# arihantb2/direct_lidar_odometry

Measured on AMD Instinct MI355X. Metric: gicp_iterations_per_sec, higher is better.
Workload: dtype f64

## Files before the change

### direct_lidar_odometry_amd/csrc/ngicp_align.h

```cpp
#pragma once

namespace {

std::mutex& persist_mutex(int device) {
  static std::mutex m[64];
  return m[(unsigned)device % 64u];
}

int pass_impl() {
  static const int impl = std::getenv("NGICP_PASS_IMPL") ? std::atoi(std::getenv("NGICP_PASS_IMPL")) : 0;
  return impl;
}

const char* robust_unsupported_switch(const ngicp* h) {
  if (pass_impl() == 1) return "NGICP_PASS_IMPL=1";
  if (const char* s = std::getenv("NGICP_FUSED")) if (std::atoi(s) != 0) return "NGICP_FUSED";
  if (const char* s = std::getenv("NGICP_QUEUE")) if (std::atoi(s) != 0) return "NGICP_QUEUE";
  if (h->persist) return "NGICP_PERSIST";
  if (h->head) return "NGICP_HEAD";
  return nullptr;
}
void refuse_if_robust(const ngicp* h, const char* entry) {
  if (h->robust_kind != NGICP_ROBUST_NONE)
    throw ArgError{NGICP_ERR_ARG, std::string(entry) + ": not available with a robust kernel set (ngicp_set_robust_kernel(h, NGICP_ROBUST_NONE, 0) turns it off)"};
}
void refuse_robust_under_switch(const ngicp* h, const char* entry) {
  if (h->robust_kind == NGICP_ROBUST_NONE) return;
  if (const char* sw = robust_unsupported_switch(h))
    throw ArgError{NGICP_ERR_ARG, std::string(entry) + ": the robust kernel has no instantiation of the pass variant " + sw + " selects (unset it, or ngicp_set_robust_kernel(h, NGICP_ROBUST_NONE, 0))"};
}
void fill_robust(const ngicp* h, int& kind, double& c, double& c2) {
  kind = h->robust_kind;
  c = h->robust_width;
  c2 = h->robust_width * h->robust_width;
}

void launch_pass(ngicp* h, const PassArgs& a, int nblocks, hipStream_t s, hipEvent_t start = nullptr, hipEvent_t stop = nullptr) {
  static const int force = std::getenv("NGICP_PASS_WPS") ? std::atoi(std::getenv("NGICP_PASS_WPS")) : 0;
  const int impl = pass_impl();
  const bool four = force ? force == 4 : nblocks > 2 * h->pass_slots;
  if (impl == 1) {
    PassArgs b = a;
    b.fused = 0;
    int need = kStGrowMax;
    if (h->p.max_corr_dist < 1e30) need = (int)std::ceil(h->p.max_corr_dist / (double)a.grid.h);
    b.stage_grow = std::max(1, std::min(kStGrowMax, need));
    if (force ? force == 4 : true)
      hipExtLaunchKernelGGL((k_gicp_pass_st<4>), dim3(nblocks), dim3(256), 0, s, start, stop, 0, b);
    else
      hipExtLaunchKernelGGL((k_gicp_pass_st<3>), dim3(nblocks), dim3(256), 0, s, start, stop, 0, b);
    return;
  }
  static const int queue_env = std::getenv("NGICP_QUEUE") ? std::atoi(std::getenv("NGICP_QUEUE")) : 0;
  if (queue_env && !a.fused && !(a.mode & 4) && !a.dbg_stamps && !a.dbg_span && !a.dbg_qstats) {
    if (four)
      hipExtLaunchKernelGGL((k_gicp_queue<2, 4>), dim3((unsigned)std::min(nblocks, h->queue_slots[1])), dim3(256), 0, s, start, stop, 0, a);
    else
      hipExtLaunchKernelGGL((k_gicp_queue<2, 3>), dim3((unsigned)std::min(nblocks, h->queue_slots[0])), dim3(256), 0, s, start, stop, 0, a);
    return;
  }
  if (a.fused) {
    if (four)
      hipExtLaunchKernelGGL((k_gicp_pass<2, 4, true>), dim3(nblocks), dim3(256), 0, s, start, stop, 0, a);
    else
      hipExtLaunchKernelGGL((k_gicp_pass<2, 3, true>), dim3(nblocks), dim3(256), 0, s, start, stop, 0, a);
    return;
  }
  if (a.robust_kind != NGICP_ROBUST_NONE) {
    if (four)
// ... 114 lines not shown
  s.cfg.lm_init_lambda_factor = h->p.lm_init_lambda_factor;
  s.partials = a.partials;
  s.nblocks = nblocks;
  s.grp_order = order_buf[h->order_sel];
  s.grp_cost = a.grp_cost;
  s.trace = own_buffers ? h->trace.as<double>() : nullptr;
  s.max_trace_rows = max_rows;
  s.mode = 0;
  s.sums_out = nullptr;
  s.dbg_stamps = nullptr;
  s.progress_host = nullptr;
  s.final_host = nullptr;
  s.order_valid = order_flag[h->order_sel];
  s.t_first = nullptr;
  s.persist = 0;
  s.pass_ticks = nullptr;
  s.st_out = nullptr;
  s.nrows = 0;
  a.crow_in = nullptr;
  a.crow_out = nullptr;
  a.cluster_ticket = nullptr;
  a.done_flag = nullptr;
  c.nblocks = nblocks;
  if (!own_buffers) return;
  h->stats.lanes_per_query = 2;
  h->stats.voxel_size = a.grid.h;
  h->stats.grid_dims[0] = a.grid.nx;
  h->stats.grid_dims[1] = a.grid.ny;
  h->stats.grid_dims[2] = a.grid.nz;
}
// ... 47 lines not shown
      for (int cc = 0; cc < 6; ++cc) hessian[cc * 6 + rr] = r.final_H[rr * 6 + cc];
  if (r.lm_failed) std::fprintf(stderr, "lm not converged!!\n");
}

void publish_alignment(ngicp* h, const LmState& st, float loop_ms, float* aligned, size_t out_stride) {
  store_result(st.hot, h->final_T, &h->converged, &h->nr_iterations, h->final_hessian);
  h->trace_host.clear();
  h->trace_rows_dev = (size_t)st.hot.n_trace;
  if (aligned) download_transformed(h, *h->src.dev, h->final_T, aligned, out_stride);
  if (st.hot.have_lin) h->hook_valid = 2;
  ngicp_stats& s = h->stats;
  s.loop_ms = loop_ms;
  s.passes = st.hot.passes;
  s.outer_iterations = st.hot.nr_iterations + 1;
  s.lm_trials = st.hot.n_trace;
  s.mean_candidates = st.hot.passes > 0 ? st.hot.cand_total / ((double)st.hot.passes * (double)h->src.dev->n) : 0.0;
  s.valid_fraction = st.hot.passes > 0 ? st.hot.valid_total / ((double)st.hot.passes * (double)h->src.dev->n) : 0.0;
  s.pass_ms_total = 0.0;
  s.passes_timed = 0;
}

void sum_event_pass_times(ngicp* h, long passes) {
  if (!h->profiling) return;
  ngicp_stats& s = h->stats;
  const long timed = std::min<long>(passes, (long)h->prof_events.size() / 2);
  int counted = 0;
  for (long i = h->prof_stride / 2; i < timed; i += h->prof_stride) {
    float ms = 0.f;
    if (hipEventElapsedTime(&ms, h->prof_events[2 * i], h->prof_events[2 * i + 1]) == hipSuccess) {
      s.pass_ms_total += ms;
      ++counted;
    }
// ... 63 lines not shown
}

void end_alignment(ngicp* h, Alignment& al, float* aligned, size_t out_stride, bool event_times = true) {
  publish_alignment(h, al.st, al.loop_ms, aligned, out_stride);
  if (event_times) sum_event_pass_times(h, al.st.hot.passes);
  ngicp_stats& s = h->stats;
  s.n_src = (long long)h->src.dev->n;
  s.n_tgt = rolling_active(h) ? (long long)h->roll.n_vox : (long long)h->tgt.dev->n;
  s.host_wait_spins = (long long)al.spins;
  s.align_ms = now_ms() - al.t_begin;
}

void set_pass_mode(const ngicp* h, PassArgs& a) {
  a.mode = (h->p.optimizer == NGICP_OPT_GAUSS_NEWTON) ? 2 : 3;
  if (h->prev_staged_fraction < 0.0 || h->prev_staged_fraction >= 0.12) a.mode |= 32;
}

bool install_xcd_order(ngicp* h, LoopCtx& c) {
  static const bool xcd_order = std::getenv("NGICP_ORDER") && std::string(std::getenv("NGICP_ORDER")) == "xcd";
  if (!xcd_order) return false;
  const int nb = c.nblocks, per = (nb + 7) / 8;
  std::vector<int> ord((size_t)nb);
  std::vector<int> lists[8];
  for (int g = 0; g < nb; ++g) lists[std::min(7, g / per)].push_back(g);
  size_t taken[8] = {0, 0, 0, 0, 0, 0, 0, 0};
  int b = 0;
  for (int placed = 0; placed < nb; ++b) {
    int x = b % 8;
    if (taken[x] >= lists[x].size()) {
      x = 0;
// ... 184 lines not shown
  pa.sa.persist = 1;
  HIP_TRY(hipMemsetAsync(pa.ticket, 0, sizeof(int), h->stream));
  HIP_TRY(hipMemsetAsync(h->gen_lines.p, 0, (size_t)kGenLines * kGenStride * sizeof(int), h->stream));
  hipExtLaunchKernelGGL((k_gicp_persist<2, 3>), dim3((unsigned)std::min(c.nblocks, h->persist_slots)), dim3(256), 0, h->stream, start, stop, 0, pa);
}

void do_align(ngicp* h, const float guess[16], float* aligned, size_t out_stride) {
  refuse_robust_under_switch(h, "ngicp_align");
  Alignment al;
  reset_results(h);
  LoopCtx c;
  prepare_loop(h, c);
  if (!(h->order_src == h->src.dev.get() && h->order_groups == c.sa.nblocks)) HIP_TRY(hipMemsetAsync(h->order_flag.p, 0, 4 * sizeof(int), h->stream));
  const bool xcd_order = install_xcd_order(h, c);
  set_pass_mode(h, c.pa);
  if (const char* dbg = std::getenv("NGICP_DEBUG_MODE")) c.pa.mode |= (std::atoi(dbg) & (8 | 16));
  begin_alignment(h, al, guess, c.sa, c.pa.t_first);
  const DebugDumps dbg = debug_begin(h, c);
  static const bool fused_env = std::getenv("NGICP_FUSED") && std::atoi(std::getenv("NGICP_FUSED")) != 0;
  if (fused_env && pass_impl() == 0) {
    c.pa.fused = 1;
    c.pa.sa = c.sa;
    HIP_TRY(hipMemsetAsync(c.pa.ticket, 0, sizeof(int), h->stream));
  }
  const long max_p = max_passes(h->p);
  const bool plain = h->p.max_iter > 0 && pass_impl() == 0 && !c.pa.fused && !xcd_order && !dbg.span_path && !dbg.qstat_path && !c.sa.dbg_stamps;
  const bool want_persist = h->persist && plain && h->persist_slots > 0 && !dbg.stamp_path && max_p + 1 <= kMaxPersistPasses;
  const bool persist_done = want_persist && align_persistent(h, c, al, max_p);
  const bool head_mode = h->head && plain && !persist_done && c.nblocks <= 2 * h->pass_slots;
  static const bool persist_one = std::getenv("NGICP_PERSIST_ONE") != nullptr;
  if (persist_done) {
  } else if (head_mode) {
    head_begin(h);
    feed_alignment(h, al, max_p + 1, [&](long i, hipEvent_t start, hipEvent_t stop) { launch_head(h, c, i, start, stop); });
    if ((al.st.hot.passes + 1) & 1) HIP_TRY(hipMemcpyAsync(h->state.p, h->state_alt.p, sizeof(LmState), hipMemcpyDeviceToDevice, h->stream));
  } else if (persist_one && h->persist_slots > 0 && max_p + 1 <= kMaxPersistPasses) {
    feed_alignment(h, al, max_p, [&](long i, hipEvent_t start, hipEvent_t stop) { launch_persist_one(h, c, i, start, stop); });
  } else {
    feed_alignment(h, al, max_p, [&](long, hipEvent_t start, hipEvent_t stop) {
      launch_pass(h, c.pa, c.nblocks, h->stream, start, stop);
      if (!c.pa.fused) hipLaunchKernelGGL(k_lm_solve, dim3(1), dim3(kSolveThreads), 0, h->stream, c.sa);
    });
  }
  HIP_TRY(hipGetLastError());
  debug_end(h, c, dbg);
  end_alignment(h, al, aligned, out_stride, !persist_done);
  ngicp_stats& s = h->stats;
  h->order_src = h->src.dev.get();
  h->order_groups = c.sa.nblocks;
  s.staged_fraction = al.st.hot.passes > 0 ? al.st.hot.staged_total / ((double)al.st.hot.passes * (double)h->src.dev->n) : 0.0;
  if (al.st.hot.passes > 1) h->prev_staged_fraction = s.staged_fraction;
  if (persist_done && h->profiling) sum_tick_pass_times(h, al.st.hot);
}

struct VoxelCtx {
  VoxelPassArgs pa;
  SolveArgs sa;
  int nblocks;
};

void launch_voxel_pass(ngicp* h, const VoxelCtx& c, hipEvent_t start = nullptr, hipEvent_t stop = nullptr) {
  const dim3 grid((unsigned)c.nblocks), block(kVoxBlock);
  if (c.pa.robust_kind != NGICP_ROBUST_NONE) {
    switch (c.pa.nbr) {
      case NGICP_VOX_DIRECT1: hipExtLaunchKernelGGL(k_vgicp_pass<true>, grid, block, 0, h->stream, start, stop, 0, c.pa); break;
      case NGICP_VOX_DIRECT7: hipExtLaunchKernelGGL((k_vgicp_pass_n<7, true>), grid, block, 0, h->stream, start, stop, 0, c.pa); break;
// ... 344 lines not shown
```

### direct_lidar_odometry_amd/csrc/ngicp_api.hip

```cpp
#include "../../include/ngicp.h"

#include <hip/hip_runtime.h>
#include <hip/hip_ext.h>

#include <algorithm>
#include <atomic>
#include <chrono>
#include <cmath>
#include <cstdio>
#include <cstdlib>
#include <cstring>
#include <limits>
#include <memory>
#include <mutex>
#include <sched.h>
#include <string>
#include <vector>

#include "ngicp_pass.h"
#include "ngicp_cloudops.h"
#include "ngicp_filters.h"
#include "ngicp_query.h"
#include "ngicp_range.h"
#include "ngicp_batch.h"
// ... 543 lines not shown
      int cus = 0, per_cu = 0;
      HIP_TRY(hipDeviceGetAttribute(&cus, hipDeviceAttributeMultiprocessorCount, device));
      HIP_TRY(hipOccupancyMaxActiveBlocksPerMultiprocessor(&per_cu, k_gicp_pass<2, 3>, 256, 0));
      h->pass_slots = std::max(1, cus) * std::max(1, per_cu);
      int per_cu_p = 0;
      if (hipOccupancyMaxActiveBlocksPerMultiprocessor(&per_cu_p, k_gicp_persist<2, 3>, 256, 0) == hipSuccess) h->persist_slots = std::max(0, cus) * std::max(0, per_cu_p);
      int q3 = 0, q4 = 0;
      if (hipOccupancyMaxActiveBlocksPerMultiprocessor(&q3, k_gicp_queue<2, 3>, 256, 0) == hipSuccess && q3 > 0) h->queue_slots[0] = cus * q3;
      if (hipOccupancyMaxActiveBlocksPerMultiprocessor(&q4, k_gicp_queue<2, 4>, 256, 0) == hipSuccess && q4 > 0) h->queue_slots[1] = cus * q4;
      int coop = 0;
      if (hipDeviceGetAttribute(&coop, hipDeviceAttributeCooperativeLaunch, device) != hipSuccess || !coop) h->persist_slots = 0;
    }
    HIP_TRY(hipHostMalloc(reinterpret_cast<void**>(&h->pin_ticks), 2 * kMaxTickPasses * sizeof(unsigned long long), hipHostMallocDefault));
    if (const char* s = std::getenv("NGICP_PERSIST")) h->persist = std::atoi(s);
    if (const char* s = std::getenv("NGICP_HEAD")) h->head = std::atoi(s);
    if (const char* s = std::getenv("NGICP_CELL_BOXES")) h->cell_boxes = std::atoi(s);
    if (const char* s = std::getenv("NGICP_TARGET_OCC")) h->target_occupancy = std::max(1.0, std::atof(s));
    if (const char* s = std::getenv("NGICP_VOXEL")) h->voxel_size = std::atof(s);
    if (const char* s = std::getenv("NGICP_CHUNK")) h->chunk_pairs = std::max(1, std::min(64, std::atoi(s)));
    if (const char* s = std::getenv("NGICP_STAGE_GROW")) h->stage_grow = std::max(0, std::min(kStageMaxGrow, std::atoi(s)));
    {
      HandleRegistry& r = registry();
      std::lock_guard<std::mutex> lock(r.m);
      r.live.push_back(h.get());
    }
    *out = h.release();
    return NGICP_OK;
  } catch (const HipError& e) {
    g_create_error = std::string("HIP error in ") + e.what + ": " + hipGetErrorString(e.code);
    (void)hipGetLastError();
// ... 794 lines not shown
    if (h->profiling && h->prof_events.empty()) {
      h->prof_events.resize(2 * 1024);
      for (auto& e : h->prof_events) HIP_TRY(hipEventCreate(&e));
    }
  });
}

int ngicp_sharded_begin(ngicp_t* h, const float guess[16]) {
  return guarded(h, [&] {
    refuse_if_voxelized(h, "ngicp_sharded_begin");
    refuse_if_robust(h, "ngicp_sharded_begin");
    h->shard_ctx.reset(new LoopCtx);
    LoopCtx& c = *h->shard_ctx;
    prepare_loop(h, c);
    set_pass_mode(h, c.pa);
    upload_initial_state(h, guess ? guess : kIdentity16);
    HIP_TRY(hipStreamSynchronize(h->stream));
    for (int i = 0; i < kShardSlots; ++i) h->h_shard_done[i] = 0;
    h->shard_steps = 0;
    h->sharded_active = true;
    h->hook_valid = 0;
  });
}

int ngicp_sharded_pass(ngicp_t* h, double* sums32_dev, void* stream_or_null) {
  return guarded(h, [&] {
    refuse_if_voxelized(h, "ngicp_sharded_pass");
    refuse_if_robust(h, "ngicp_sharded_pass");
    if (!h->sharded_active || !h->shard_ctx) throw ArgError{NGICP_ERR_STATE, "ngicp_sharded_begin not called"};
    if (!sums32_dev) throw ArgError{NGICP_ERR_ARG, "null sums buffer"};
// ... 38 lines not shown
    }
    if (done) *done = d;
  });
}

int ngicp_sharded_finish(ngicp_t* h, float T_out[16], int* converged, int* nr_iterations, double final_hessian[36]) {
  return guarded(h, [&] {
    refuse_if_voxelized(h, "ngicp_sharded_finish");
    refuse_if_robust(h, "ngicp_sharded_finish");
    if (!h->sharded_active) throw ArgError{NGICP_ERR_STATE, "ngicp_sharded_begin not called"};
    hipStream_t s = h->shard_stream ? h->shard_stream : h->stream;
    HIP_TRY(hipMemcpyAsync(&h->pin_state[1], h->state.p, sizeof(LmState), hipMemcpyDeviceToHost, s));
    HIP_TRY(hipStreamSynchronize(s));
    store_result(h->pin_state[1].hot, h->final_T, &h->converged, &h->nr_iterations, h->final_hessian);
    copy_results_out(h, T_out, converged, nr_iterations, final_hessian);
    h->sharded_active = false;
    h->shard_ctx.reset();
    h->shard_stream = nullptr;
  });
}

int ngicp_covs_shard_begin(ngicp_t* h, int which, double** covs6_dev, size_t* n_points) {
  return guarded(h, [&] {
    refuse_if_voxelized(h, "ngicp_covs_shard_begin");
    if ((which != 0 && which != 1) || !covs6_dev || !n_points) throw ArgError{NGICP_ERR_ARG, "bad argument"};
    Slot& slot = which ? h->tgt : h->src;
    ensure_slot_ready(h, slot, which ? "target" : "source");
    CovSet& cs = h->shard_covs[which];
    cs.data = acquire_buf(h, h->device, slot.dev->n * 6 * sizeof(double));
    cs.n = slot.dev->n;
// ... 415 lines not shown
```

### direct_lidar_odometry_amd/csrc/ngicp_handle.h

```cpp
#pragma once

namespace {

thread_local std::string g_create_error;

struct HipError {
  hipError_t code;
  const char* what;
  const char* file;
  int line;
};

#define HIP_TRY(expr)                                          \
  do {                                                         \
    hipError_t _e = (expr);                                    \
    if (_e != hipSuccess) throw HipError{_e, #expr, __FILE__, __LINE__}; \
  } while (0)

struct ArgError {
  int code;
  std::string msg;
};

double now_ms() {
// ... 241 lines not shown
  int prof_stride = 1;

  Slot src, tgt;
  CovSet src_covs, tgt_covs;

  DevBuf raw, unsorted, keys, counts, fill, tile_sums, tile_sq, tmp, bbox, occ;
  int pass_slots = 768;
  int persist_slots = 0;
  int queue_slots[2] = {768, 1024};
  int persist = 0;
  int order_sel = 0;
  DevBuf grp_order_alt;
  DevBuf gen_lines;
  int cell_boxes = 0;
  int head = 0;
  DevBuf state_alt;
  DevBuf head_ws;
  unsigned long long* pin_ticks = nullptr;
  double prev_staged_fraction = -1.0;
  DevBuf dbg, dbg_q, dbg_s, dbg_span, grp_order, grp_cost, batch_far;
  const void* order_src = nullptr;
  int order_groups = -1;
  DevBuf tpt[2], mahal[2], partials, state, trace, tfinal, out_xyz, scratch16, queries, knn_idx, knn_d2, sums, ticket;
  DevBuf fit_T, fit_part, fit_out, rad_counts, rad_offsets, rad_keys, rad_long;
  size_t rad_total = 0;
  bool rad_valid = false;
  DevBuf range_ws;
  hipEvent_t ev_q_a = nullptr, ev_q_b = nullptr;
  std::vector<hipEvent_t> prof_events;
  int* h_progress = nullptr;
// ... 124 lines not shown
```

### direct_lidar_odometry_amd/csrc/ngicp_pass.h

```cpp
#pragma once
#include <type_traits>

#include "../../include/ngicp.h"
#include "ngicp_knn.h"

namespace ngk {

constexpr int kPartialStride = 32;
constexpr int kNumSums = 29;
constexpr int kNumSlots = 32;
constexpr int kTraceCols = 8;

__device__ __forceinline__ void lin_terms(double (&acc)[kNumSums], const double tax, const double tay, const double taz, const double ex, const double ey, const double ez,
                                          const double (&M)[6]) {
  const double m00 = M[0], m01 = M[1], m02 = M[2], m11 = M[3], m12 = M[4], m22 = M[5];
  const double mex = m00 * ex + m01 * ey + m02 * ez;
  const double mey = m01 * ex + m11 * ey + m12 * ez;
  const double mez = m02 * ex + m12 * ey + m22 * ez;
  acc[27] += ex * mex + ey * mey + ez * mez;
  const double A00 = tay * m02 - taz * m01, A10 = taz * m00 - tax * m02, A20 = tax * m01 - tay * m00;
  const double A01 = tay * m12 - taz * m11, A11 = taz * m01 - tax * m12, A21 = tax * m11 - tay * m01;
  const double A02 = tay * m22 - taz * m12, A12 = taz * m02 - tax * m22, A22 = tax * m12 - tay * m02;
  acc[0] += -(A01 * taz - A02 * tay);
  acc[1] += -(-A00 * taz + A02 * tax);
// ... 84 lines not shown
  double staged_total;
  int iter;
  int trial;
  int have_lin;
  int cur;
  int done;
  int converged;
  int nr_iterations;
  int lm_failed;
  int n_trace;
  int passes;
  int pending;
  double final_H[36];
  unsigned long long t_first, t_done;
  float lin_f[12];
};
constexpr int kViewXi = 0;
constexpr int kViewXiF = 24;
constexpr int kViewDone = 36, kViewCur = 37, kViewHaveLin = 38;
struct LmState {
  LmHot hot;
  float xi_f[12];
  alignas(512) int view[128];
};
constexpr int kViewWords = 128;
constexpr int kGenLines = 256, kGenStride = 32;
static_assert(sizeof(LmState) % 512 == 0 && offsetof(LmState, view) % 512 == 0, "ring entries are 512-byte aligned");

struct PassPose {
  double R[9], t[3];
// ... 52 lines not shown
  int nblocks;
  double* trace;
  int max_trace_rows;
  int mode;
  double* sums_out;
  int* grp_order;
  const int* grp_cost;
  unsigned long long* dbg_stamps;
  int* progress_host;
  LmHot* final_host;
  int* order_valid;
  const unsigned long long* t_first;
  LmState* st_out;
  int nrows;
  int persist;
  unsigned long long* pass_ticks;
};

struct PassArgs {
  const float4* qpts;
  const int2* batches;
  const float* batch_boxes;
  const int* grp_order;
  int* grp_cost;
  int n_batches;
  const double* cov_src;
  int n_src;
  const float4* tgt;
  const float4* tgtp;
  const Xyz* tgt3;
// ... 317 lines not shown
  for (int i = 0; i < 36; ++i) A[i] = L.H[i];
#pragma unroll
  for (int i = 0; i < 6; ++i) {
    A[i * 6 + i] += lambda_add;
    rhs[i] = -L.b[i];
  }
  ldlt6_solve(A, rhs, L.d);
  pose_identity(L.delta);
  so3_exp_matrix(L.d, L.delta.R);
  L.delta.t[0] = L.d[3];
  L.delta.t[1] = L.d[4];
  L.delta.t[2] = L.d[5];
  pose_mul(L.delta, L.x0, L.xi);
}

__device__ __forceinline__ void adopt_new(LmHot& L, const double* sums) {
#pragma unroll
  for (int r = 0; r < 6; ++r)
#pragma unroll
    for (int c = r; c < 6; ++c) L.H[r * 6 + c] = L.H[c * 6 + r] = sums[tri21(r, c)];
#pragma unroll
  for (int i = 0; i < 6; ++i) L.b[i] = sums[21 + i];
  L.y0 = sums[27];
  L.cur ^= 1;
  L.have_lin = 1;
#pragma unroll
  for (int r = 0; r < 3; ++r) {
#pragma unroll
    for (int c = 0; c < 3; ++c) L.lin_f[r * 4 + c] = (float)L.xi.R[r * 3 + c];
    L.lin_f[r * 4 + 3] = (float)L.xi.t[r];
// ... 23 lines not shown
    L.nr_iterations = 0;
    if (L.lambda < 0.0) {
      double m = 0.0;
#pragma unroll
      for (int i = 0; i < 6; ++i) m = fmax(m, fabs(L.H[i * 6 + i]));
      L.lambda = cfg.lm_init_lambda_factor * m;
    }
    L.nu = 2.0;
    L.trial = 0;
    if (cfg.lm_max_iterations <= 0) {
      L.lm_failed = 1;
      L.done = 1;
      return false;
    }
    make_trial(L, L.lambda);
    return false;
  }

  double den = 0.0, dn = 0.0;
#pragma unroll
  for (int i = 0; i < 6; ++i) {
    den += L.d[i] * (L.lambda * L.d[i] - L.b[i]);
    dn += L.d[i] * L.d[i];
  }
  const double rho = (L.y0 - yi) / den;
  const bool rejected = rho < 0;
  if (trace && L.n_trace < max_trace_rows) {
    double* row = trace + (size_t)L.n_trace * kTraceCols;
    row[0] = L.iter; row[1] = L.trial; row[2] = L.y0; row[3] = yi;
    row[4] = rho; row[5] = L.lambda; row[6] = sqrt(dn); row[7] = rejected ? 0.0 : 1.0;
// ... 3 lines not shown
    if (is_converged_dev(L.delta, cfg.rot_eps, cfg.trans_eps)) {
      L.converged = 1;
      L.done = 1;
      return false;
    }
    L.lambda = L.nu * L.lambda;
    L.nu = 2 * L.nu;
    L.trial += 1;
    if (L.trial >= cfg.lm_max_iterations) {
      L.lm_failed = 1;
      L.converged = 0;
      L.done = 1;
      return false;
    }
    make_trial(L, L.lambda);
    return false;
  }
  return true;
}

__device__ __forceinline__ void lm_step(LmHot& L, const LmConfig& cfg, const double* sums, double* trace, int max_trace_rows) {
  const bool gn = cfg.optimizer == 0;
  const bool accepted = lm_advance(L, cfg, sums, trace, max_trace_rows);
  if (accepted) {
#pragma unroll
    for (int i = 0; i < 36; ++i) L.final_H[i] = L.H[i];
    if (!gn) {
      double den = 0.0;
#pragma unroll
      for (int i = 0; i < 6; ++i) den += L.d[i] * (L.lambda * L.d[i] - L.b[i]);
      const double rho = (L.y0 - sums[28]) / den;
      L.x0 = L.xi;
      const double q = 2 * rho - 1;
      L.lambda = L.lambda * fmax(1.0 / 3.0, 1 - q * q * q);
      L.converged = is_converged_dev(L.delta, cfg.rot_eps, cfg.trans_eps) ? 1 : 0;
      L.iter += 1;
      if (L.converged || L.iter >= cfg.max_iterations) {
        L.done = 1;
      } else {
        adopt_new(L, sums);
        L.nr_iterations = L.iter;
        L.nu = 2.0;
        L.trial = 0;
        make_trial(L, L.lambda);
      }
    }
  }
  if (gn && !L.done) L.xi = L.x0;
}

template <int THREADS>
struct SolveShared {
  double wsum[32][kPartialStride];
  double sums[kPartialStride];
  int ord_cnt[THREADS / 64 - 1][16], ord_pos[THREADS / 64 - 1][16];
  int ord_cost[kMaxOrderGroups];
  unsigned char ord_cls[kMaxOrderGroups];
  int ord_arrived;
  LmHot L;
// ... 20 lines not shown
  LmState* st = a.st;
  LmState* sto = a.st_out ? a.st_out : a.st;
#define NG_SSTAMP(k)                                                                 \
  do {                                                                               \
    if (a.dbg_stamps && threadIdx.x == 0) a.dbg_stamps[k] = __builtin_amdgcn_s_memtime(); \
  } while (0)
  const int done_at_entry = PERSIST ? 0 : __hip_atomic_load(&st->hot.done, __ATOMIC_RELAXED, __HIP_MEMORY_SCOPE_WORKGROUP);
  const unsigned long long t_solver_entry = a.dbg_stamps ? __builtin_amdgcn_s_memtime() : 0ull;
  const int lane = threadIdx.x & 63, wave = threadIdx.x >> 6;
  const int vp = threadIdx.x & 15, sb = threadIdx.x >> 4;
  const double2* __restrict__ rows = reinterpret_cast<const double2*>(a.partials) + vp;
  static_assert(sizeof(LmHot) % 4 == 0, "LmHot is copied as dwords");
  constexpr int kHotWords = (int)(sizeof(LmHot) / 4), kHotPerThread = (kHotWords + kSolveThreads - 1) / kSolveThreads;
  constexpr int kCostPerThread = kMaxOrderGroups / kSolveThreads;
  const int passes_at_entry = PERSIST ? __hip_atomic_load(&st->hot.passes, __ATOMIC_RELAXED, __HIP_MEMORY_SCOPE_AGENT) : st->hot.passes;
  const bool order_it = a.mode == 0 && a.grp_order && a.nblocks <= kMaxOrderGroups && (PERSIST ? passes_at_entry == 2 : (!AGENT || passes_at_entry < 3 || (passes_at_entry & 3) == 3));
  int hv[kHotPerThread];
#pragma unroll
  for (int k = 0; k < kHotPerThread; ++k) {
    const int w = threadIdx.x + k * kSolveThreads;
    if constexpr (PERSIST) hv[k] = w < kHotWords ? __hip_atomic_load(reinterpret_cast<const int*>(&st->hot) + w, __ATOMIC_RELAXED, __HIP_MEMORY_SCOPE_AGENT) : 0;
    else hv[k] = w < kHotWords ? reinterpret_cast<const int*>(&st->hot)[w] : 0;
  }
  const int last_row = (a.nrows ? a.nrows : a.nblocks) - 1, last_grp = a.nblocks - 1;
  auto load_row = [](const double2* q) -> double2 {
    if constexpr (PERSIST) {
      const double* d = reinterpret_cast<const double*>(q);
      return make_double2(__hip_atomic_load(d, __ATOMIC_RELAXED, __HIP_MEMORY_SCOPE_AGENT), __hip_atomic_load(d + 1, __ATOMIC_RELAXED, __HIP_MEMORY_SCOPE_AGENT));
    } else {
      return *q;
    }
// ... 146 lines not shown
      if (sw == 0 && lane == 0 && a.order_valid) *a.order_valid = 1;
    }
    if (a.dbg_stamps && sw == 0 && lane == 0) a.dbg_stamps[7] = __builtin_amdgcn_s_memtime() - t_ord;
  }
  if (wave != 0) return;
  if (a.mode == 2) {
    if (lane == 0) st->hot.y0 = sums[28];
    return;
  }
  if (lane == 0) {
    if (a.mode == 1) {
      adopt_new(L, sums);
    } else {
      const LmConfig& cfg = a.cfg;
      NG_SSTAMP(3);
      lm_step(L, cfg, sums, a.trace, a.max_trace_rows);
      NG_SSTAMP(4);
      NG_SSTAMP(5);
      if (!L.done) {
#pragma unroll
        for (int r = 0; r < 3; ++r) {
#pragma unroll
          for (int c = 0; c < 4; ++c) {
            const float f = (float)(c < 3 ? L.xi.R[r * 3 + c] : L.xi.t[r]);
            if constexpr (PERSIST) __hip_atomic_store(&st->xi_f[r * 4 + c], f, __ATOMIC_RELAXED, __HIP_MEMORY_SCOPE_AGENT);
            else sto->xi_f[r * 4 + c] = f;
          }
        }
      }
    }
  }
// ... 56 lines not shown
  static_assert(kWin <= kSortedPad, "walk windows may overhang the array by at most the sentinel frame");
  static_assert(B == kBatchQueries, "query batches are built for 32 queries (2 lanes per query)");
  __shared__ double lds[4][kNumSlots];
  struct Nothing {};
  union PassShared {
    WaveStage stage[4];
    typename std::conditional<FUSED, SolveShared<256>, Nothing>::type sv;
  };
  __shared__ PassShared shm;
  __shared__ int last_block;
  WaveStage* stage_all = shm.stage;
  const LmState* __restrict__ st = a.st;
  typedef const int __attribute__((address_space(4))) * ConstIntPtr;
  const int done_now = st->hot.done, have_lin_now = st->hot.have_lin;
  const int cur = st->hot.cur, nxt = cur ^ 1;
  const int order_is_valid = *(ConstIntPtr)(unsigned long long)a.order_valid;
  const int order_entry = ((ConstIntPtr)(unsigned long long)a.grp_order)[blockIdx.x];
  double R[9], t[3];
#pragma unroll
  for (int i = 0; i < 9; ++i) R[i] = st->hot.xi.R[i];
#pragma unroll
  for (int i = 0; i < 3; ++i) t[i] = st->hot.xi.t[i];
  float Tf[12];
#pragma unroll
  for (int i = 0; i < 12; ++i) Tf[i] = st->xi_f[i];
  asm volatile("" ::"s"(done_now), "s"(have_lin_now), "s"(cur), "s"(order_is_valid), "s"(order_entry), "s"(Tf[0]), "s"(Tf[11]), "s"(R[0]), "s"(t[2]));
  if (!(a.mode & 4) && done_now) return;

  const bool do_err = (a.mode & 1) && have_lin_now;
  const bool do_lin = (a.mode & 2);
  const float4* __restrict__ tpt_old = a.tpt[cur];
  const double* __restrict__ mahal_old = a.mahal[cur];
  float4* __restrict__ tpt_new = a.tpt[nxt];
  double* __restrict__ mahal_new = a.mahal[nxt];
  const Grid& g = a.grid;

  double wave_total = 0.0;
  unsigned int ncand = 0, nvalid = 0, nstaged = 0;

  const int lane = threadIdx.x & 63, wave = __builtin_amdgcn_readfirstlane((int)(threadIdx.x >> 6));
  const int sub = lane % G, grp = lane / G;
  WaveStage& S = stage_all[wave];
  NG_STAMP(0);
  const int group = order_is_valid ? order_entry : (int)blockIdx.x;
  const unsigned long long t_start = a.grp_cost ? __builtin_amdgcn_s_memtime() : 0ull;
  if (a.dbg_span && threadIdx.x == 0) a.dbg_span[(size_t)blockIdx.x * 4] = __builtin_amdgcn_s_memrealtime();
  if (a.t_first && blockIdx.x == 0 && threadIdx.x == 0 && !have_lin_now) *a.t_first = __builtin_amdgcn_s_memrealtime();
#define NG_HAVE_LIN have_lin_now
#define NG_ROBUST ROBUST
#include "ngicp_pass_group.inc"
#undef NG_ROBUST
#undef NG_HAVE_LIN
  if constexpr (FUSED) {
  if (wave == 0) {
    asm volatile("s_waitcnt vmcnt(0)" ::: "memory");
    if (lane == 0) {
      const int tk = __hip_atomic_fetch_add(a.ticket, 1, __ATOMIC_RELAXED, __HIP_MEMORY_SCOPE_AGENT);
      last_block = (tk == (int)gridDim.x - 1) ? 1 : 0;
    }
  }
  __syncthreads();
  if (!last_block) return;
  if (threadIdx.x == 0) {
    __hip_atomic_store(a.ticket, 0, __ATOMIC_RELAXED, __HIP_MEMORY_SCOPE_AGENT);
    __builtin_amdgcn_fence(__ATOMIC_ACQUIRE, "agent");
    asm volatile("s_waitcnt vmcnt(0)" ::: "memory");
  }
// ... 336 lines not shown
```

### direct_lidar_odometry_amd/nano_gicp.py

```python
from __future__ import annotations

import ctypes as C
import enum
import os
import sys

import numpy as np

_HERE = os.path.dirname(os.path.abspath(__file__))
_LIB_PATH = os.environ.get("NGICP_LIB") or os.path.join(_HERE, "libngicp_hip.so")

c_f32p = C.POINTER(C.c_float)
c_f64p = C.POINTER(C.c_double)
c_i32p = C.POINTER(C.c_int)

FLT_MAX = float(np.finfo(np.float32).max)


class RegularizationMethod(enum.IntEnum):
    NONE = 0
    MIN_EIG = 1
    NORMALIZED_MIN_EIG = 2
    PLANE = 3
    FROBENIUS = 4
# ... 17 lines not shown
    GEMAN_MCCLURE = 3


class NgicpError(RuntimeError):
    def __init__(self, code: int, msg: str):
        super().__init__(f"ngicp error {code}: {msg}")
        self.code = code


class Stats(C.Structure):
    _fields_ = [("align_ms", C.c_double), ("loop_ms", C.c_double), ("pass_ms_total", C.c_double), ("passes", C.c_int),
                ("outer_iterations", C.c_int), ("lm_trials", C.c_int), ("mean_candidates", C.c_double), ("valid_fraction", C.c_double),
                ("index_build_ms", C.c_double), ("covariance_ms", C.c_double), ("upload_ms", C.c_double), ("voxel_size", C.c_double),
                ("grid_dims", C.c_int * 3), ("lanes_per_query", C.c_int), ("passes_timed", C.c_int), ("n_src", C.c_longlong), ("n_tgt", C.c_longlong), ("staged_fraction", C.c_double), ("submap_ms", C.c_double),
                ("device_allocs", C.c_longlong), ("host_wait_spins", C.c_longlong), ("query_ms", C.c_double),
                ("voxelmap_ms", C.c_double)]

    def as_dict(self):
        d = {k: getattr(self, k) for k, _ in self._fields_}
        d["grid_dims"] = list(self.grid_dims)
        return d


EXPORTS = [
    "ngicp_create", "ngicp_destroy", "ngicp_last_error", "ngicp_version", "ngicp_set_params", "ngicp_set_tuning",
    "ngicp_set_source", "ngicp_register_source", "ngicp_set_target", "ngicp_clear_source", "ngicp_clear_target",
    "ngicp_share_source_index", "ngicp_swap_source_target", "ngicp_compute_source_covs", "ngicp_compute_target_covs",
    "ngicp_copy_source_covs", "ngicp_clear_source_covs", "ngicp_clear_target_covs", "ngicp_source_covs_size",
    "ngicp_target_covs_size", "ngicp_get_source_covs", "ngicp_get_target_covs", "ngicp_set_source_covs",
    "ngicp_set_target_covs", "ngicp_align", "ngicp_linearize", "ngicp_compute_error", "ngicp_get_correspondences",
    "ngicp_target_knn", "ngicp_get_lm_trace", "ngicp_get_stats", "ngicp_set_profiling", "ngicp_sharded_begin",
# ... 687 lines not shown
```

### include/ngicp.h

```cpp
#ifndef NGICP_H
#define NGICP_H

#include <stddef.h>
#include <stdint.h>

#ifdef __cplusplus
extern "C" {
#endif

typedef struct ngicp ngicp_t;

#define NGICP_OK 0
#define NGICP_ERR_HIP (-1)
#define NGICP_ERR_ARG (-2)
#define NGICP_ERR_STATE (-3)
#define NGICP_ERR_K_TOO_LARGE (-4)

#define NGICP_REG_NONE 0
#define NGICP_REG_MIN_EIG 1
#define NGICP_REG_NORMALIZED_MIN_EIG 2
#define NGICP_REG_PLANE 3
#define NGICP_REG_FROBENIUS 4

#define NGICP_OPT_GAUSS_NEWTON 0
// ... 95 lines not shown
  double valid_fraction;
  double index_build_ms;
  double covariance_ms;
  double upload_ms;
  double voxel_size;
  int grid_dims[3];
  int lanes_per_query;
  int passes_timed;
  long long n_src, n_tgt;
  double staged_fraction;
  double submap_ms;
  long long device_allocs;
  long long host_wait_spins;
  double query_ms;
  double voxelmap_ms;
} ngicp_stats;
int ngicp_get_stats(ngicp_t* h, ngicp_stats* out);
int ngicp_set_profiling(ngicp_t* h, int on);

int ngicp_sharded_begin(ngicp_t* h, const float guess_colmajor[16]);
int ngicp_sharded_pass(ngicp_t* h, double* sums32_dev, void* hip_stream_or_null);
int ngicp_sharded_step(ngicp_t* h, const double* sums32_dev, void* hip_stream_or_null, int* done);
int ngicp_sharded_finish(ngicp_t* h, float T_out_colmajor[16], int* converged, int* nr_iterations, double final_hessian_colmajor[36]);
int ngicp_covs_shard_begin(ngicp_t* h, int which, double** covs6_dev, size_t* n_points);
int ngicp_covs_shard_compute(ngicp_t* h, int which, size_t lo, size_t hi, void* hip_stream_or_null);
int ngicp_covs_shard_commit(ngicp_t* h, int which);

int ngicp_keyframe_add(ngicp_t* h, ngicp_t* from, int* id_out);
int ngicp_keyframe_add_transformed(ngicp_t* h, ngicp_t* from, const float T_colmajor[16], int* id_out);
int ngicp_keyframe_add_transformed_filtered(ngicp_t* h, ngicp_t* from, const float T_colmajor[16], float leaf, int* id_out);
// ... 26 lines not shown
```

Baseline: 20130.

## Skip correspondence search on final LM trial when linearization is not needed

Adds a device-side lin_unneeded flag, set when the trial step will converge or hit the iteration cap. When the flag is set, the pass kernel skips the neighbour search and Hessian accumulation. It only evaluates the error term against the previous correspondences and Mahalanobis matrices. This is meant to remove a full search/linearize pass at the end of each alignment, at the cost of evaluating the final cost with stale correspondences, which can change acceptance behaviour slightly. Stats now count search passes separately.

```diff
diff --git a/direct_lidar_odometry_amd/csrc/ngicp_align.h b/direct_lidar_odometry_amd/csrc/ngicp_align.h
--- a/direct_lidar_odometry_amd/csrc/ngicp_align.h
+++ b/direct_lidar_odometry_amd/csrc/ngicp_align.h
@@ -33,6 +33,11 @@
   kind = h->robust_kind;
   c = h->robust_width;
   c2 = h->robust_width * h->robust_width;
+}
+
+int queue_switch() {
+  static const int queue_env = std::getenv("NGICP_QUEUE") ? std::atoi(std::getenv("NGICP_QUEUE")) : 0;
+  return queue_env;
 }
 
 void launch_pass(ngicp* h, const PassArgs& a, int nblocks, hipStream_t s, hipEvent_t start = nullptr, hipEvent_t stop = nullptr) {
@@ -51,8 +56,7 @@
       hipExtLaunchKernelGGL((k_gicp_pass_st<3>), dim3(nblocks), dim3(256), 0, s, start, stop, 0, b);
     return;
   }
-  static const int queue_env = std::getenv("NGICP_QUEUE") ? std::atoi(std::getenv("NGICP_QUEUE")) : 0;
-  if (queue_env && !a.fused && !(a.mode & 4) && !a.dbg_stamps && !a.dbg_span && !a.dbg_qstats) {
+  if (queue_switch() && !a.fused && !(a.mode & 4) && !a.dbg_stamps && !a.dbg_span && !a.dbg_qstats) {
     if (four)
       hipExtLaunchKernelGGL((k_gicp_queue<2, 4>), dim3((unsigned)std::min(nblocks, h->queue_slots[1])), dim3(256), 0, s, start, stop, 0, a);
     else
@@ -197,6 +201,7 @@
   s.order_valid = order_flag[h->order_sel];
   s.t_first = nullptr;
   s.persist = 0;
+  s.pass_honours_word = 0;
   s.pass_ticks = nullptr;
   s.st_out = nullptr;
   s.nrows = 0;
@@ -274,8 +279,9 @@
   s.passes = st.hot.passes;
   s.outer_iterations = st.hot.nr_iterations + 1;
   s.lm_trials = st.hot.n_trace;
-  s.mean_candidates = st.hot.passes > 0 ? st.hot.cand_total / ((double)st.hot.passes * (double)h->src.dev->n) : 0.0;
-  s.valid_fraction = st.hot.passes > 0 ? st.hot.valid_total / ((double)st.hot.passes * (double)h->src.dev->n) : 0.0;
+  s.search_passes = st.hot.search_passes;
+  s.mean_candidates = st.hot.search_passes > 0 ? st.hot.cand_total / ((double)st.hot.search_passes * (double)h->src.dev->n) : 0.0;
+  s.valid_fraction = st.hot.search_passes > 0 ? st.hot.valid_total / ((double)st.hot.search_passes * (double)h->src.dev->n) : 0.0;
   s.pass_ms_total = 0.0;
   s.passes_timed = 0;
 }
@@ -369,6 +375,12 @@
 void set_pass_mode(const ngicp* h, PassArgs& a) {
   a.mode = (h->p.optimizer == NGICP_OPT_GAUSS_NEWTON) ? 2 : 3;
   if (h->prev_staged_fraction < 0.0 || h->prev_staged_fraction >= 0.12) a.mode |= 32;
+}
+
+void honour_lin_unneeded(const ngicp* h, LoopCtx& c) {
+  if (h->full_last_pass || pass_impl() != 0 || queue_switch()) return;
+  c.pa.mode |= 64;
+  c.sa.pass_honours_word = 1;
 }
 
 bool install_xcd_order(ngicp* h, LoopCtx& c) {
@@ -583,6 +595,8 @@
   if (!(h->order_src == h->src.dev.get() && h->order_groups == c.sa.nblocks)) HIP_TRY(hipMemsetAsync(h->order_flag.p, 0, 4 * sizeof(int), h->stream));
   const bool xcd_order = install_xcd_order(h, c);
   set_pass_mode(h, c.pa);
+  static const bool persist_one = std::getenv("NGICP_PERSIST_ONE") != nullptr;
+  if (!h->persist && !h->head && !persist_one) honour_lin_unneeded(h, c);
   if (const char* dbg = std::getenv("NGICP_DEBUG_MODE")) c.pa.mode |= (std::atoi(dbg) & (8 | 16));
   begin_alignment(h, al, guess, c.sa, c.pa.t_first);
   const DebugDumps dbg = debug_begin(h, c);
@@ -597,7 +611,6 @@
   const bool want_persist = h->persist && plain && h->persist_slots > 0 && !dbg.stamp_path && max_p + 1 <= kMaxPersistPasses;
   const bool persist_done = want_persist && align_persistent(h, c, al, max_p);
   const bool head_mode = h->head && plain && !persist_done && c.nblocks <= 2 * h->pass_slots;
-  static const bool persist_one = std::getenv("NGICP_PERSIST_ONE") != nullptr;
   if (persist_done) {
   } else if (head_mode) {
     head_begin(h);
@@ -617,8 +630,8 @@
   ngicp_stats& s = h->stats;
   h->order_src = h->src.dev.get();
   h->order_groups = c.sa.nblocks;
-  s.staged_fraction = al.st.hot.passes > 0 ? al.st.hot.staged_total / ((double)al.st.hot.passes * (double)h->src.dev->n) : 0.0;
-  if (al.st.hot.passes > 1) h->prev_staged_fraction = s.staged_fraction;
+  s.staged_fraction = al.st.hot.search_passes > 0 ? al.st.hot.staged_total / ((double)al.st.hot.search_passes * (double)h->src.dev->n) : 0.0;
+  if (al.st.hot.search_passes > 1) h->prev_staged_fraction = s.staged_fraction;
   if (persist_done && h->profiling) sum_tick_pass_times(h, al.st.hot);
 }
 
diff --git a/direct_lidar_odometry_amd/csrc/ngicp_api.hip b/direct_lidar_odometry_amd/csrc/ngicp_api.hip
--- a/direct_lidar_odometry_amd/csrc/ngicp_api.hip
+++ b/direct_lidar_odometry_amd/csrc/ngicp_api.hip
@@ -581,6 +581,7 @@
     HIP_TRY(hipHostMalloc(reinterpret_cast<void**>(&h->pin_ticks), 2 * kMaxTickPasses * sizeof(unsigned long long), hipHostMallocDefault));
     if (const char* s = std::getenv("NGICP_PERSIST")) h->persist = std::atoi(s);
     if (const char* s = std::getenv("NGICP_HEAD")) h->head = std::atoi(s);
+    if (const char* s = std::getenv("NGICP_FULL_LAST_PASS")) h->full_last_pass = std::atoi(s);
     if (const char* s = std::getenv("NGICP_CELL_BOXES")) h->cell_boxes = std::atoi(s);
     if (const char* s = std::getenv("NGICP_TARGET_OCC")) h->target_occupancy = std::max(1.0, std::atof(s));
     if (const char* s = std::getenv("NGICP_VOXEL")) h->voxel_size = std::atof(s);
@@ -1405,6 +1406,7 @@
     LoopCtx& c = *h->shard_ctx;
     prepare_loop(h, c);
     set_pass_mode(h, c.pa);
+    honour_lin_unneeded(h, c);
     upload_initial_state(h, guess ? guess : kIdentity16);
     HIP_TRY(hipStreamSynchronize(h->stream));
     for (int i = 0; i < kShardSlots; ++i) h->h_shard_done[i] = 0;
@@ -1473,6 +1475,9 @@
     HIP_TRY(hipStreamSynchronize(s));
     store_result(h->pin_state[1].hot, h->final_T, &h->converged, &h->nr_iterations, h->final_hessian);
     copy_results_out(h, T_out, converged, nr_iterations, final_hessian);
+    h->stats.passes = h->pin_state[1].hot.passes;
+    h->stats.search_passes = h->pin_state[1].hot.search_passes;
+    h->stats.lm_trials = h->pin_state[1].hot.n_trace;
     h->sharded_active = false;
     h->shard_ctx.reset();
     h->shard_stream = nullptr;
diff --git a/direct_lidar_odometry_amd/csrc/ngicp_handle.h b/direct_lidar_odometry_amd/csrc/ngicp_handle.h
--- a/direct_lidar_odometry_amd/csrc/ngicp_handle.h
+++ b/direct_lidar_odometry_amd/csrc/ngicp_handle.h
@@ -279,6 +279,7 @@
   DevBuf gen_lines;
   int cell_boxes = 0;
   int head = 0;
+  int full_last_pass = 0;
   DevBuf state_alt;
   DevBuf head_ws;
   unsigned long long* pin_ticks = nullptr;
diff --git a/direct_lidar_odometry_amd/csrc/ngicp_pass.h b/direct_lidar_odometry_amd/csrc/ngicp_pass.h
--- a/direct_lidar_odometry_amd/csrc/ngicp_pass.h
+++ b/direct_lidar_odometry_amd/csrc/ngicp_pass.h
@@ -122,6 +122,8 @@
   double final_H[36];
   unsigned long long t_first, t_done;
   float lin_f[12];
+  int lin_unneeded;
+  int search_passes;
 };
 constexpr int kViewXi = 0;
 constexpr int kViewXiF = 24;
@@ -204,6 +206,7 @@
   LmState* st_out;
   int nrows;
   int persist;
+  int pass_honours_word;
   unsigned long long* pass_ticks;
 };
 
@@ -551,6 +554,10 @@
   pose_mul(L.delta, L.x0, L.xi);
 }
 
+__device__ __forceinline__ void set_lin_unneeded(LmHot& L, const LmConfig& cfg) {
+  L.lin_unneeded = (is_converged_dev(L.delta, cfg.rot_eps, cfg.trans_eps) || L.iter + 1 >= cfg.max_iterations) ? 1 : 0;
+}
+
 __device__ __forceinline__ void adopt_new(LmHot& L, const double* sums) {
 #pragma unroll
   for (int r = 0; r < 6; ++r)
@@ -604,6 +611,7 @@
       return false;
     }
     make_trial(L, L.lambda);
+    set_lin_unneeded(L, cfg);
     return false;
   }
 
@@ -637,13 +645,15 @@
       return false;
     }
     make_trial(L, L.lambda);
+    set_lin_unneeded(L, cfg);
     return false;
   }
   return true;
 }
 
-__device__ __forceinline__ void lm_step(LmHot& L, const LmConfig& cfg, const double* sums, double* trace, int max_trace_rows) {
+__device__ __forceinline__ void lm_step(LmHot& L, const LmConfig& cfg, const double* sums, double* trace, int max_trace_rows, const bool searched = true) {
   const bool gn = cfg.optimizer == 0;
+  L.search_passes += searched ? 1 : 0;
   const bool accepted = lm_advance(L, cfg, sums, trace, max_trace_rows);
   if (accepted) {
 #pragma unroll
@@ -666,6 +676,7 @@
         L.nu = 2.0;
         L.trial = 0;
         make_trial(L, L.lambda);
+        set_lin_unneeded(L, cfg);
       }
     }
   }
@@ -716,7 +727,8 @@
   constexpr int kHotWords = (int)(sizeof(LmHot) / 4), kHotPerThread = (kHotWords + kSolveThreads - 1) / kSolveThreads;
   constexpr int kCostPerThread = kMaxOrderGroups / kSolveThreads;
   const int passes_at_entry = PERSIST ? __hip_atomic_load(&st->hot.passes, __ATOMIC_RELAXED, __HIP_MEMORY_SCOPE_AGENT) : st->hot.passes;
-  const bool order_it = a.mode == 0 && a.grp_order && a.nblocks <= kMaxOrderGroups && (PERSIST ? passes_at_entry == 2 : (!AGENT || passes_at_entry < 3 || (passes_at_entry & 3) == 3));
+  const int k4_only_at_entry = (!PERSIST && a.pass_honours_word) ? st->hot.lin_unneeded : 0;
+  const bool order_it = a.mode == 0 && a.grp_order && a.nblocks <= kMaxOrderGroups && !k4_only_at_entry && (PERSIST ? passes_at_entry == 2 : (!AGENT || passes_at_entry < 3 || (passes_at_entry & 3) == 3));
   int hv[kHotPerThread];
 #pragma unroll
   for (int k = 0; k < kHotPerThread; ++k) {
@@ -893,7 +905,7 @@
     } else {
       const LmConfig& cfg = a.cfg;
       NG_SSTAMP(3);
-      lm_step(L, cfg, sums, a.trace, a.max_trace_rows);
+      lm_step(L, cfg, sums, a.trace, a.max_trace_rows, !(a.pass_honours_word && L.lin_unneeded));
       NG_SSTAMP(4);
       NG_SSTAMP(5);
       if (!L.done) {
@@ -980,6 +992,7 @@
   typedef const int __attribute__((address_space(4))) * ConstIntPtr;
   const int done_now = st->hot.done, have_lin_now = st->hot.have_lin;
   const int cur = st->hot.cur, nxt = cur ^ 1;
+  const int lin_unneeded_now = st->hot.lin_unneeded;
   const int order_is_valid = *(ConstIntPtr)(unsigned long long)a.order_valid;
   const int order_entry = ((ConstIntPtr)(unsigned long long)a.grp_order)[blockIdx.x];
   double R[9], t[3];
@@ -990,7 +1003,7 @@
   float Tf[12];
 #pragma unroll
   for (int i = 0; i < 12; ++i) Tf[i] = st->xi_f[i];
-  asm volatile("" ::"s"(done_now), "s"(have_lin_now), "s"(cur), "s"(order_is_valid), "s"(order_entry), "s"(Tf[0]), "s"(Tf[11]), "s"(R[0]), "s"(t[2]));
+  asm volatile("" ::"s"(done_now), "s"(have_lin_now), "s"(cur), "s"(lin_unneeded_now), "s"(order_is_valid), "s"(order_entry), "s"(Tf[0]), "s"(Tf[11]), "s"(R[0]), "s"(t[2]));
   if (!(a.mode & 4) && done_now) return;
 
   const bool do_err = (a.mode & 1) && have_lin_now;
@@ -1012,11 +1025,71 @@
   const unsigned long long t_start = a.grp_cost ? __builtin_amdgcn_s_memtime() : 0ull;
   if (a.dbg_span && threadIdx.x == 0) a.dbg_span[(size_t)blockIdx.x * 4] = __builtin_amdgcn_s_memrealtime();
   if (a.t_first && blockIdx.x == 0 && threadIdx.x == 0 && !have_lin_now) *a.t_first = __builtin_amdgcn_s_memrealtime();
+  if ((a.mode & 64) && lin_unneeded_now) {
+    const int item = group * 4 + wave;
+    double term = 0.0;
+    if (item < a.n_batches) {
+      typedef const int __attribute__((address_space(4))) * ConstBatchPtr;
+      ConstBatchPtr brec = (ConstBatchPtr)(unsigned long long)a.batches + 2 * (size_t)item;
+      const int qbase = brec[0], qcount = brec[1];
+      if (lane < qcount) {
+        const int i = qbase + lane;
+        const float4 sp = a.qpts[i];
+        float4 bp_old = make_float4(0.f, 0.f, 0.f, 0.f);
+        int j_old = -1;
+        double Mold[6] = {0, 0, 0, 0, 0, 0};
+        if (have_lin_now) {
+          bp_old = tpt_old[i];
+          j_old = __float_as_int(bp_old.w);
+        }
+        if (do_err) {
+          const double* M = mahal_old + (size_t)i * 6;
+#pragma unroll
+          for (int e = 0; e < 6; ++e) Mold[e] = M[e];
+        }
+        double k4 = 0.0;
+        if (do_err && j_old >= 0) {
+          const double ax = (double)sp.x, ay = (double)sp.y, az = (double)sp.z;
+          const double tax = R[0] * ax + R[1] * ay + R[2] * az + t[0];
+          const double tay = R[3] * ax + R[4] * ay + R[5] * az + t[1];
+          const double taz = R[6] * ax + R[7] * ay + R[8] * az + t[2];
+          const double ex = (double)bp_old.x - tax, ey = (double)bp_old.y - tay, ez = (double)bp_old.z - taz;
+          if constexpr (ROBUST) k4 = err_term_robust(a.robust_kind, a.robust_c, a.robust_c2, ex, ey, ez, Mold);
+          else k4 = err_term(ex, ey, ez, Mold);
+        }
+        term += k4;
+      }
+    }
+    double* red = S.red;
+    if (lane < 32) red[lane] = term;
+    wave_lds_sync();
+    if (lane < kNumSlots) {
+      double out = 0.0;
+      if (lane == 28)
+        for (int l = 0; l < 32; ++l) out += red[l];
+      wave_total += out;
+      lds[wave][lane] = lane == 28 ? wave_total : 0.0;
+    }
+    __syncthreads();
+    if (threadIdx.x < kNumSlots) {
+      const int v = threadIdx.x;
+      const double val = ((lds[0][v] + lds[1][v]) + lds[2][v]) + lds[3][v];
+      if (FUSED) __hip_atomic_store(a.partials + (size_t)group * kNumSlots + v, val, __ATOMIC_RELAXED, __HIP_MEMORY_SCOPE_AGENT);
+      else a.partials[(size_t)group * kNumSlots + v] = val;
+    }
+    if (a.dbg_span && threadIdx.x == 0) {
+      unsigned long long* d = a.dbg_span + (size_t)blockIdx.x * 4;
+      d[1] = __builtin_amdgcn_s_memrealtime();
+      d[3] = (unsigned long long)(unsigned int)group;
+    }
+    if constexpr (!FUSED) return;
+  } else {
 #define NG_HAVE_LIN have_lin_now
 #define NG_ROBUST ROBUST
 #include "ngicp_pass_group.inc"
 #undef NG_ROBUST
 #undef NG_HAVE_LIN
+  }
   if constexpr (FUSED) {
   if (wave == 0) {
     asm volatile("s_waitcnt vmcnt(0)" ::: "memory");
diff --git a/direct_lidar_odometry_amd/nano_gicp.py b/direct_lidar_odometry_amd/nano_gicp.py
--- a/direct_lidar_odometry_amd/nano_gicp.py
+++ b/direct_lidar_odometry_amd/nano_gicp.py
@@ -55,7 +55,7 @@
                 ("index_build_ms", C.c_double), ("covariance_ms", C.c_double), ("upload_ms", C.c_double), ("voxel_size", C.c_double),
                 ("grid_dims", C.c_int * 3), ("lanes_per_query", C.c_int), ("passes_timed", C.c_int), ("n_src", C.c_longlong), ("n_tgt", C.c_longlong), ("staged_fraction", C.c_double), ("submap_ms", C.c_double),
                 ("device_allocs", C.c_longlong), ("host_wait_spins", C.c_longlong), ("query_ms", C.c_double),
-                ("voxelmap_ms", C.c_double)]
+                ("voxelmap_ms", C.c_double), ("search_passes", C.c_int)]
 
     def as_dict(self):
         d = {k: getattr(self, k) for k, _ in self._fields_}
diff --git a/include/ngicp.h b/include/ngicp.h
--- a/include/ngicp.h
+++ b/include/ngicp.h
@@ -133,6 +133,7 @@
   long long host_wait_spins;
   double query_ms;
   double voxelmap_ms;
+  int search_passes;
 } ngicp_stats;
 int ngicp_get_stats(ngicp_t* h, ngicp_stats* out);
 int ngicp_set_profiling(ngicp_t* h, int on);
```

Result: faster. 20450 (median of 6 runs) (+1.6%).
